# miuda-ai/lele

Hardware: AMD Instinct MI355X
Metric: STFT+mel GB/s (SenseVoice front-end: PCM -> log-mel -> LFR, algorithmic bytes); SenseVoiceSmall-shaped RTF in `sensevoice` (higher is better)
Workload: dtype f32

## Files before the change

### lele_amd/csrc/fe_core.h

```cpp
#pragma once
#include <stdint.h>

#if defined(__HIPCC__)
#define FE_HD __host__ __device__ __forceinline__
#else
#define FE_HD inline
#endif

namespace fe {

constexpr int kNfft = 512;
constexpr int kFrame = 400;
constexpr int kHop = 160;
constexpr int kBins = 257;
constexpr int kLanes = 16;
constexpr int kRegs = 32;
constexpr int kQ = 25;

FE_HD constexpr int rev4(int x) { return ((x & 1) << 3) | ((x & 2) << 1) | ((x & 4) >> 1) | ((x & 8) >> 3); }
FE_HD constexpr int rev5(int x) {
    return ((x & 1) << 4) | ((x & 2) << 2) | (x & 4) | ((x & 8) >> 2) | ((x & 16) >> 4);
}
FE_HD constexpr int tw_off(int s) { return (1 << (s - 1)) - 1; }

FE_HD float fmul(float a, float b) { return a * b; }
FE_HD float fadd(float a, float b) { return a + b; }
FE_HD float fsub(float a, float b) { return a - b; }
FE_HD float ffma(float a, float b, float c) { return __builtin_fmaf(a, b, c); }

#if defined(__HIPCC__) && defined(__HIP_DEVICE_COMPILE__)
typedef float cf __attribute__((ext_vector_type(2)));
FE_HD cf cmk(float re, float im) { return (cf){re, im}; }
FE_HD cf cadd(cf a, cf b) { return a + b; }
FE_HD cf csub(cf a, cf b) { return a - b; }
FE_HD cf cmulv(cf a, cf b) { return a * b; }
FE_HD cf cfmav(cf a, cf b, cf c) { return __builtin_elementwise_fma(a, b, c); }
FE_HD cf cswap(cf a) { return a.yx; }
FE_HD cf cxx(cf a) { return a.xx; }
#else
struct cf {
    float x, y;
};
FE_HD cf cmk(float re, float im) { return cf{re, im}; }
FE_HD cf cadd(cf a, cf b) { return cf{a.x + b.x, a.y + b.y}; }
FE_HD cf csub(cf a, cf b) { return cf{a.x - b.x, a.y - b.y}; }
FE_HD cf cmulv(cf a, cf b) { return cf{a.x * b.x, a.y * b.y}; }
FE_HD cf cfmav(cf a, cf b, cf c) { return cf{__builtin_fmaf(a.x, b.x, c.x), __builtin_fmaf(a.y, b.y, c.y)}; }
FE_HD cf cswap(cf a) { return cf{a.y, a.x}; }
FE_HD cf cxx(cf a) { return cf{a.x, a.x}; }
#endif

struct Tw {
    cf w, wn;
};
FE_HD Tw make_tw(float wr, float wi) { return Tw{cmk(wr, wi), cmk(-wi, wi)}; }

FE_HD cf tw_mul_fma(const Tw& t, cf o) { return cfmav(cxx(t.w), o, cmulv(t.wn, cswap(o))); }

FE_HD void bfly_fma(const Tw& tw, cf& e, cf& o) {
    cf t = tw_mul_fma(tw, o);
    cf n = csub(e, t);
    e = cadd(e, t);
    o = n;
}
FE_HD void bfly_scalar(float wr, float wi, cf& e, cf& o) {
    float tr = fsub(fmul(wr, o.x), fmul(wi, o.y));
    float ti = fadd(fmul(wr, o.y), fmul(wi, o.x));
    cf t = cmk(tr, ti);
    cf n = csub(e, t);
    e = cadd(e, t);
    o = n;
}
FE_HD void bfly_fma(float wr, float wi, float& er, float& ei, float& o_r, float& oi) {
    cf e = cmk(er, ei), o = cmk(o_r, oi);
    bfly_fma(make_tw(wr, wi), e, o);
    er = e.x;
    ei = e.y;
    o_r = o.x;
    oi = o.y;
}
FE_HD void bfly_scalar(float wr, float wi, float& er, float& ei, float& o_r, float& oi) {
    cf e = cmk(er, ei), o = cmk(o_r, oi);
    bfly_scalar(wr, wi, e, o);
    er = e.x;
    ei = e.y;
    o_r = o.x;
    oi = o.y;
}

template <typename TW>
FE_HD void phase_a(cf* a, const TW& tw_re, const TW& tw_im) {
#pragma unroll
    for (int r = 0; r < kRegs; r += 2) bfly_scalar(tw_re[tw_off(1)], tw_im[tw_off(1)], a[r], a[r + 1]);
#pragma unroll
    for (int b = 0; b < kRegs; b += 4) {
#pragma unroll
        for (int k = 0; k < 2; ++k) bfly_scalar(tw_re[tw_off(2) + k], tw_im[tw_off(2) + k], a[b + k], a[b + 2 + k]);
    }
#pragma unroll
    for (int s = 3; s <= 5; ++s) {
        const int half = 1 << (s - 1);
#pragma unroll
        for (int b = 0; b < kRegs; b += 2 * half) {
#pragma unroll
            for (int k = 0; k < half; ++k)
                bfly_fma(make_tw(tw_re[tw_off(s) + k], tw_im[tw_off(s) + k]), a[b + k], a[b + half + k]);
        }
    }
}

template <typename TW>
FE_HD void phase_a_fast(const float* x, cf* a, const TW& tw_re, const TW& tw_im) {
    float s1[kRegs];
#pragma unroll
    for (int r = 0; r < kRegs; r += 2) {
        if (rev5(r + 1) >= kQ) {
            s1[r] = x[r];
            s1[r + 1] = x[r];
        } else {
            s1[r] = fadd(x[r], x[r + 1]);
            s1[r + 1] = fsub(x[r], x[r + 1]);
        }
    }
    {
        const float wr = tw_re[tw_off(2) + 1], wi = tw_im[tw_off(2) + 1];
#pragma unroll
        for (int b = 0; b < kRegs; b += 4) {
            a[b] = cmk(fadd(s1[b], s1[b + 2]), 0.0f);
            a[b + 2] = cmk(fsub(s1[b], s1[b + 2]), 0.0f);
            const float tr = fmul(wr, s1[b + 3]);
            const float ti = fmul(wi, s1[b + 3]);
            a[b + 1] = cmk(fadd(s1[b + 1], tr), ti);
            a[b + 3] = cmk(fsub(s1[b + 1], tr), -ti);
        }
    }
#pragma unroll
    for (int b = 0; b < kRegs; b += 8) {
#pragma unroll
        for (int k = 0; k < 4; ++k) {
            const float wr = tw_re[tw_off(3) + k], wi = tw_im[tw_off(3) + k];
            if ((k & 1) == 0) {
                const float e = a[b + k].x, o = a[b + 4 + k].x;
                const float tr = fmul(wr, o);
                const float ti = fmul(wi, o);
                a[b + k] = cmk(fadd(e, tr), ti);
                a[b + 4 + k] = cmk(fsub(e, tr), -ti);
            } else {
                bfly_fma(make_tw(wr, wi), a[b + k], a[b + 4 + k]);
            }
        }
    }
#pragma unroll
    for (int s = 4; s <= 5; ++s) {
        const int half = 1 << (s - 1);
#pragma unroll
        for (int b = 0; b < kRegs; b += 2 * half) {
#pragma unroll
            for (int k = 0; k < half; ++k)
                bfly_fma(make_tw(tw_re[tw_off(s) + k], tw_im[tw_off(s) + k]), a[b + k], a[b + half + k]);
        }
    }
}

template <typename TWF>
FE_HD void phase_b(cf* b, int c, int rho, const TWF& twf, float* re256) {
#pragma unroll
    for (int s = 6; s <= 8; ++s) {
        const int hv = 1 << (s - 6);
#pragma unroll
        for (int k = 0; k < hv; ++k) {
            const cf w = twf(tw_off(s) + k * 32 + rho * 16 + c);
            const Tw tw = make_tw(w.x, w.y);
#pragma unroll
            for (int base = 0; base < 16; base += 2 * hv) bfly_fma(tw, b[base + k], b[base + hv + k]);
        }
    }
#pragma unroll
    for (int k = 0; k < 8; ++k) {
        const cf w = twf(tw_off(9) + k * 32 + rho * 16 + c);
        const cf t = tw_mul_fma(make_tw(w.x, w.y), b[8 + k]);
        if (k == 0) *re256 = fsub(b[0].x, t.x);
        b[k] = cadd(b[k], t);
    }
}

FE_HD float power(float re, float im) { return fadd(fmul(re, re), fmul(im, im)); }
FE_HD float power(cf z) {
    cf sq = cmulv(z, z);
    return fadd(sq.x, sq.y);
}

constexpr int kXchgPitch = 17;
FE_HD constexpr int xchg_slot(int v, int c) { return v * kXchgPitch + c; }

}
```

### lele_amd/csrc/frontend.hip

```cpp
#include <type_traits>
#include "common.h"
#include "fe_core.h"

#include <math.h>

#include <algorithm>

using namespace lele;

namespace {

constexpr int kMaxMelRounds = 8;

struct FeDev {
    const float* tw_re;
    const float* tw_im;
    const float2* tw;
    const float* window;
    const float* melw;
    const int* mel_start;
    const int* mel_step_off;
    int mel_rounds;
    int mel_steps;
    int n_mels;
    int lfr_m, lfr_n;
};

struct GridBlock {
    __device__ __forceinline__ unsigned x() const { return blockIdx.x; }
    __device__ __forceinline__ unsigned y() const { return blockIdx.y; }
};
struct SegBlock {
    unsigned bx;
    __device__ __forceinline__ unsigned x() const { return bx; }
    __device__ __forceinline__ unsigned y() const { return 0u; }
};

struct FeSeg {
    int64_t start, len;
    int64_t num_frames, t_lfr;
    int64_t row0;
    int64_t block0;
};

constexpr int kSumRows = 66;
constexpr int kSumPitch = 164;

__global__ __launch_bounds__(64) void fe_frame_sum_kernel(const float* __restrict__ pcm, int64_t utt_stride,
                                                          int64_t pcm_len, int64_t num_frames,
                                                          float* __restrict__ mean_out, int aligned16) {
    __shared__ __attribute__((aligned(16))) float tile[kSumRows * kSumPitch];
    const int lane = threadIdx.x;
    const int64_t f0 = (int64_t)blockIdx.x * 64;
    const float* base = pcm + (int64_t)blockIdx.y * utt_stride;
    const int64_t s0 = f0 * fe::kHop;
    constexpr int kVecPerRow = fe::kHop / 4;
    constexpr int kVecs = kSumRows * kVecPerRow;
    constexpr int kIters = (kVecs + 63) / 64;
    constexpr int kBatch = 14;
    static_assert(kIters % kBatch == 0, "batching");
    for (int b0 = 0; b0 < kIters; b0 += kBatch) {
        float4 st[kBatch];
#pragma unroll
        for (int u = 0; u < kBatch; ++u) {
            const int idx = (b0 + u) * 64 + lane;
            int64_t s = s0 + 4 * (int64_t)idx;
            if (s + 3 >= pcm_len) s = aligned16 ? ((pcm_len - 4) & ~int64_t(3)) : (pcm_len - 4);
            if (s < 0) s = 0;
            const float* src = base + s;
            if (aligned16) {
                st[u] = *reinterpret_cast<const float4*>(src);
            } else {
                st[u] = make_float4(src[0], src[1], src[2], src[3]);
            }
        }
#pragma unroll
        for (int u = 0; u < kBatch; ++u) {
            const int idx = (b0 + u) * 64 + lane;
            if (idx < kVecs) {
                float4 xv = st[u];
                xv.x *= 32768.0f;
                xv.y *= 32768.0f;
                xv.z *= 32768.0f;
                xv.w *= 32768.0f;
                const int row = idx / kVecPerRow, c = idx - row * kVecPerRow;
                *reinterpret_cast<float4*>(&tile[row * kSumPitch + 4 * c]) = xv;
            }
        }
    }
    __syncthreads();
    float sum = 0.0f;
#pragma unroll
    for (int seg = 0; seg < 3; ++seg) {
        const float* rowp = &tile[(lane + seg) * kSumPitch];
        const int nvec = seg < 2 ? kVecPerRow : (fe::kFrame - 2 * fe::kHop) / 4;
#pragma unroll 10
        for (int k = 0; k < nvec; ++k) {
            const float4 r = *reinterpret_cast<const float4*>(rowp + 4 * k);
            sum = sum + r.x;
            sum = sum + r.y;
            sum = sum + r.z;
            sum = sum + r.w;
        }
    }
    const int64_t f = f0 + lane;
    if (f < num_frames) mean_out[(int64_t)blockIdx.y * num_frames + f] = sum / (float)fe::kFrame;
}

constexpr int kFrameXchgFloats = 2 * 16 * fe::kXchgPitch;
constexpr int kWaveLdsFloats = 4 * kFrameXchgFloats;
constexpr int kPStride = 272;

struct TwLds {
    const float2* t;
    __device__ __forceinline__ float2 at(int i) const { return t[i]; }
};

template <int MODE>
__device__ __forceinline__ float lane_rot_prev(float v, int p) {
    if (MODE == 1) {
        return __builtin_bit_cast(float,
                                  __builtin_amdgcn_update_dpp(0, __builtin_bit_cast(int, v), 0x121, 0xf, 0xf, true));
    } else {
        return __shfl(v, (p + 15) & 15, 16);
    }
}

constexpr int kStdMelLen[5] = {3, 4, 6, 10, 17};
constexpr int kStdMelOff[6] = {0, 3, 7, 13, 23, 40};

template <int MODE, bool STDMEL, bool FUSED, int PASSES, bool LOWREG, class Blk>
__device__ __forceinline__ void fe_main_body(const float* __restrict__ pcm, int64_t utt_stride,
                                             int64_t num_frames, int64_t t_lfr,
                                             const float* __restrict__ means, const FeDev& tb,
                                             float* __restrict__ out, float* __restrict__ logmel_out,
                                             int aligned16, float* s_melw, Blk bl) {
    constexpr int FR = 16 * PASSES;
    constexpr int kRows = FR + 2;
    constexpr int kXFloats = FUSED ? (kRows * kSumPitch > 4 * kWaveLdsFloats ? kRows * kSumPitch : 4 * kWaveLdsFloats)
                                   : 4 * kWaveLdsFloats;
    __shared__ float2 s_tw[LOWREG ? 480 : 512];
    __shared__ __attribute__((aligned(16))) float s_x[kXFloats];
    __shared__ float s_mean[64];
    __shared__ int s_mstart[16 * (STDMEL ? 5 : kMaxMelRounds)];
    __shared__ int s_moff[kMaxMelRounds + 1];
    constexpr int kTwBase = LOWREG ? 31 : 0;

    for (int i = threadIdx.x; i < 511 - kTwBase; i += 256) s_tw[i] = tb.tw[i + kTwBase];
    if (!STDMEL)
        for (int i = threadIdx.x; i < tb.mel_steps * 16; i += 256) s_melw[i] = tb.melw[i];
    if (threadIdx.x < tb.mel_rounds * 16) s_mstart[threadIdx.x] = tb.mel_start[threadIdx.x];
    if (threadIdx.x <= tb.mel_rounds) s_moff[threadIdx.x] = tb.mel_step_off[threadIdx.x];
    const int lane = threadIdx.x & 63, wave = threadIdx.x >> 6;
    const int g = lane >> 4, p = lane & 15;
    if (FUSED) {
        const float* ubase = pcm + (int64_t)bl.y() * utt_stride;
        const int64_t s0 = (int64_t)bl.x() * FR * fe::kHop;
        constexpr int kVecPerRow = fe::kHop / 4;
        constexpr int kVecs = kRows * kVecPerRow;
        constexpr int kIters = (kVecs + 255) / 256;
        float4 st[kIters];
#pragma unroll
        for (int u = 0; u < kIters; ++u) {
            const int idx = u * 256 + (int)threadIdx.x;
            int64_t sidx = s0 + 4 * (int64_t)idx;
            if (sidx + 3 >= utt_stride) sidx = aligned16 ? ((utt_stride - 4) & ~int64_t(3)) : (utt_stride - 4);
            if (sidx < 0) sidx = 0;
            const float* src = ubase + sidx;
            if (aligned16)
                st[u] = *reinterpret_cast<const float4*>(src);
            else
                st[u] = make_float4(src[0], src[1], src[2], src[3]);
        }
#pragma unroll
        for (int u = 0; u < kIters; ++u) {
            const int idx = u * 256 + (int)threadIdx.x;
            if (idx < kVecs) {
                float4 xv = st[u];
                xv.x *= 32768.0f;
                xv.y *= 32768.0f;
                xv.z *= 32768.0f;
                xv.w *= 32768.0f;
                const int row = idx / kVecPerRow, c = idx - row * kVecPerRow;
                *reinterpret_cast<float4*>(&s_x[row * kSumPitch + 4 * c]) = xv;
            }
        }
        __syncthreads();
    }
    const int h = fe::rev4(p);
    float* xw = s_x + wave * kWaveLdsFloats;
    float* xf = xw + g * kFrameXchgFloats;
    const float* base = pcm + (int64_t)bl.y() * utt_stride;
    const float* mean_u = means + (int64_t)bl.y() * num_frames;
    const int d_out = tb.n_mels * tb.lfr_m;
    float* out_u = out ? out + (int64_t)bl.y() * t_lfr * d_out : nullptr;
    float* lm_u = logmel_out ? logmel_out + (int64_t)bl.y() * num_frames * tb.n_mels : nullptr;

    float win[fe::kQ];
    if (!LOWREG) {
#pragma unroll
        for (int q = 0; q < fe::kQ; ++q) win[q] = tb.window[p + 16 * q];
    }

    float xr[fe::kQ];
    float mean_next = 0.0f;
    auto issue_loads = [&](int pass) {
        const int64_t f = (int64_t)bl.x() * FR + wave * (4 * PASSES) + pass * 4 + g;
        const int64_t fc = f < num_frames ? f : 0;
        const float* src = base + fc * fe::kHop + p;
        if (!FUSED) mean_next = mean_u[fc];
#pragma unroll
        for (int q = 0; q < fe::kQ; ++q) xr[q] = src[16 * q];
    };
    issue_loads(0);
    if (FUSED) {
        constexpr int kVecPerRow = fe::kHop / 4;
        if (wave == 0 && lane < FR) {
            float sum = 0.0f;
#pragma unroll
            for (int seg = 0; seg < 3; ++seg) {
                const float* rowp = &s_x[(lane + seg) * kSumPitch];
                const int nvec = seg < 2 ? kVecPerRow : (fe::kFrame - 2 * fe::kHop) / 4;
#pragma unroll 10
                for (int k = 0; k < nvec; ++k) {
                    const float4 r = *reinterpret_cast<const float4*>(rowp + 4 * k);
                    sum = sum + r.x;
                    sum = sum + r.y;
                    sum = sum + r.z;
                    sum = sum + r.w;
                }
            }
            s_mean[lane] = sum / (float)fe::kFrame;
        }
    }
    __syncthreads();

    auto run_pass = [&](int pass, auto load_next_c) {
        constexpr bool load_next = decltype(load_next_c)::value;
        const int64_t f = (int64_t)bl.x() * FR + wave * (4 * PASSES) + pass * 4 + g;
        const bool valid = f < num_frames;
        const float mean = FUSED ? s_mean[wave * (4 * PASSES) + pass * 4 + g] : mean_next;
        if (LOWREG) {
            int off = 0;
            asm volatile("" : "+v"(off));
#pragma unroll
            for (int q = 0; q < fe::kQ; ++q) win[q] = tb.window[p + 16 * q + off];
        }

        float v[fe::kQ];
        const float neg_mean = -mean;
#pragma unroll
        for (int q = 0; q < fe::kQ; ++q) v[q] = __builtin_fmaf(xr[q], 32768.0f, neg_mean);
        if (load_next) issue_loads(pass + 1);
        float xin[fe::kRegs];
#pragma unroll
        for (int r = 0; r < fe::kRegs; ++r) xin[r] = 0.0f;
        float k97;
        asm("v_mov_b32 %0, 0x3f7851ec" : "=v"(k97));
#pragma unroll
        for (int q = 0; q < fe::kQ; ++q) {
            const float send = (p == 15 && q > 0) ? v[q > 0 ? q - 1 : 0] : v[q];
            const float prev = lane_rot_prev<MODE>(send, p);
            float y = fe::fsub(v[q], fe::fmul(k97, prev));
            if (q == 0) y = (p == 0) ? v[0] : y;
            xin[fe::rev5(q)] = fe::fmul(y, win[q]);
        }

        fe::cf a[fe::kRegs];
        fe::phase_a_fast(xin, a, tb.tw_re, tb.tw_im);

        float pw[2][8];
        float p256 = 0.0f;
#pragma unroll
        for (int rho = 0; rho < 2; ++rho) {
            __builtin_amdgcn_wave_barrier();
#pragma unroll
            for (int cc = 0; cc < 16; ++cc) {
                const int slot = fe::xchg_slot(h, cc);
                *reinterpret_cast<float2*>(xf + 2 * slot) = make_float2(a[rho * 16 + cc].x, a[rho * 16 + cc].y);
            }
            __builtin_amdgcn_wave_barrier();
            fe::cf bq[16];
#pragma unroll
            for (int vv = 0; vv < 16; ++vv) {
                const float2 t = *reinterpret_cast<const float2*>(xf + 2 * fe::xchg_slot(vv, p));
                bq[vv] = fe::cmk(t.x, t.y);
            }
            __builtin_amdgcn_wave_barrier();
            float re256 = 0.0f;
            fe::phase_b(bq, p, rho, [&](int i) { const float2 w = s_tw[i - kTwBase]; return fe::cmk(w.x, w.y); }, &re256);
            if (rho == 0) p256 = re256;
#pragma unroll
            for (int vv = 0; vv < 8; ++vv) {
                fe::cf z = bq[vv];
                if (vv == 0 && rho == 0) z = fe::cmk(z.x, (p == 0) ? 0.0f : z.y);
                pw[rho][vv] = fe::power(z);
            }
        }
        float* prow = xw + g * kPStride;
        __builtin_amdgcn_wave_barrier();
#pragma unroll
        for (int rho = 0; rho < 2; ++rho)
#pragma unroll
            for (int vv = 0; vv < 8; ++vv) prow[(2 * vv + rho) * 16 + p] = pw[rho][vv];
        if (p == 0) prow[256] = fe::power(p256, 0.0f);
        __builtin_amdgcn_wave_barrier();

        const int fi = (int)f, nfr = (int)num_frames, tl = (int)t_lfr;
        const int pad = (tb.lfr_m - 1) / 2;
        const int fp = fi + pad;
        const int b_first = fp % tb.lfr_n, i_first = fp / tb.lfr_n;

        float vals[STDMEL ? 5 : kMaxMelRounds];
#pragma unroll
        for (int rd = 0; rd < (STDMEL ? 5 : kMaxMelRounds); ++rd) {
            vals[rd] = 0.0f;
            if (!STDMEL && rd >= tb.mel_rounds) continue;
            const int m = rd * 16 + p;
            const int start = s_mstart[m];
            const float* pp = prow + start;
            float acc = 0.0f;
            if (STDMEL) {
                const float* wp = tb.melw + kStdMelOff[rd < 5 ? rd : 0] * 16 + p;
                float w[17];
#pragma unroll
                for (int t = 0; t < 17; ++t)
                    if (t < kStdMelLen[rd < 5 ? rd : 0]) w[t] = wp[t * 16];
#pragma unroll
                for (int t = 0; t < 17; ++t)
                    if (t < kStdMelLen[rd < 5 ? rd : 0]) acc = fe::fadd(acc, fe::fmul(w[t], pp[t]));
            } else {
                const int t0 = s_moff[rd], t1 = s_moff[rd + 1];
                const float* wp = s_melw + t0 * 16 + p;
                const int lim = 256 - start;
#pragma unroll 4
                for (int t = 0; t < t1 - t0; ++t) {
                    const float pv = pp[t < lim ? t : lim];
                    acc = fe::fadd(acc, fe::fmul(wp[t * 16], pv));
                }
            }
            {
                const float l2 = __builtin_amdgcn_logf(fmaxf(acc, 1e-5f));
                const float hi = __builtin_bit_cast(float, 0x3f317217u), lo = __builtin_bit_cast(float, 0x3377d1cfu);
                const float r = fe::fmul(l2, hi);
                vals[rd] = fe::fadd(r, fe::ffma(l2, lo, fe::ffma(l2, hi, -r)));
            }
        }
        if (valid) {
            constexpr int kR = STDMEL ? 5 : kMaxMelRounds;
            auto put = [&](float* dst) {
#pragma unroll
                for (int rd = 0; rd < kR; ++rd)
                    if (rd * 16 + p < tb.n_mels) __builtin_nontemporal_store(vals[rd], &dst[rd * 16]);
            };
            if (lm_u) put(lm_u + (int64_t)fi * tb.n_mels + p);
            if (out_u) {
                int i = i_first;
                for (int b = b_first; b < tb.lfr_m && i >= 0; b += tb.lfr_n, --i)
                    if (i < tl) put(out_u + i * d_out + b * tb.n_mels + p);
                if (fi == 0) {
                    for (int i2 = 0; i2 * tb.lfr_n - pad < 0 && i2 < tl; ++i2)
                        for (int b = 0; b < tb.lfr_m && i2 * tb.lfr_n + b - pad < 0; ++b)
                            put(out_u + i2 * d_out + b * tb.n_mels + p);
                }
                if (fi == nfr - 1) {
                    for (int i2 = tl - 1; i2 >= 0 && i2 * tb.lfr_n + (tb.lfr_m - 1) - pad > fi; --i2)
                        for (int b = tb.lfr_m - 1; b >= 0 && i2 * tb.lfr_n + b - pad > fi; --b)
                            put(out_u + i2 * d_out + b * tb.n_mels + p);
                }
            }
        }
        __builtin_amdgcn_wave_barrier();
    };
#pragma unroll 1
    for (int pass = 0; pass + 1 < PASSES; ++pass) run_pass(pass, std::true_type{});
    run_pass(PASSES - 1, std::false_type{});
}

template <int MODE, bool STDMEL, bool FUSED>
__global__ __launch_bounds__(256) void fe_main_kernel(const float* __restrict__ pcm, int64_t utt_stride, int64_t num_frames, int64_t t_lfr,
                                                      const float* __restrict__ means, FeDev tb, float* __restrict__ out,
                                                      float* __restrict__ logmel_out, int aligned16) {
    extern __shared__ float s_melw[];
    fe_main_body<MODE, STDMEL, FUSED, 4, false>(pcm, utt_stride, num_frames, t_lfr, means, tb, out, logmel_out, aligned16, s_melw,
                                                GridBlock{});
}

template <int MODE, bool STDMEL>
__global__ __launch_bounds__(256) void fe_seg_main_kernel(const float* __restrict__ pcm, const FeSeg* __restrict__ segs,
                                                          const int* __restrict__ blk_seg, FeDev tb, float* __restrict__ out) {
    extern __shared__ float s_melw[];
    const FeSeg s = segs[blk_seg[blockIdx.x]];
    const float* base = pcm + s.start;
    const int aligned16 = (((uintptr_t)base & 15) == 0) && (s.len % 4 == 0);
    fe_main_body<MODE, STDMEL, true, 4, false>(base, s.len, s.num_frames, s.t_lfr, nullptr, tb, out + s.row0 * (tb.n_mels * tb.lfr_m),
                                               nullptr, aligned16, s_melw, SegBlock{(unsigned)(blockIdx.x - s.block0)});
}
__global__ void fe_generic_mean_kernel(const float* __restrict__ pcm, int64_t rows, int64_t num_frames, int64_t pcm_len, int frame_len, int hop,
                                       float* __restrict__ mean) {
    const int64_t f = (int64_t)blockIdx.x * blockDim.x + threadIdx.x;
    if (f >= rows) return;
    const float* src = pcm + (f / num_frames) * pcm_len + (f % num_frames) * hop;
    float sum = 0.0f;
    int j = 0;
    if ((((uintptr_t)src) & 15) == 0) {
        for (; j + 16 <= frame_len; j += 16) {
            float4 v[4];
#pragma unroll
            for (int u = 0; u < 4; ++u) v[u] = *reinterpret_cast<const float4*>(src + j + 4 * u);
#pragma unroll
            for (int u = 0; u < 4; ++u) {
                sum = sum + v[u].x * 32768.0f;
                sum = sum + v[u].y * 32768.0f;
                sum = sum + v[u].z * 32768.0f;
                sum = sum + v[u].w * 32768.0f;
            }
        }
    }
    for (; j < frame_len; ++j) sum = sum + src[j] * 32768.0f;
    mean[f] = sum / (float)frame_len;
}
__global__ void fe_generic_frame_kernel(const float* __restrict__ pcm, const float* __restrict__ mean,
                                        const float* __restrict__ window, int64_t rows, int64_t num_frames, int64_t pcm_len, int frame_len, int hop,
                                        int n_fft, float* __restrict__ frames) {
    const int64_t total = rows * n_fft;
    for (int64_t i = (int64_t)blockIdx.x * blockDim.x + threadIdx.x; i < total; i += (int64_t)gridDim.x * blockDim.x) {
        const int64_t f = i / n_fft;
        const int j = (int)(i - f * n_fft);
        float v = 0.0f;
        if (j < frame_len) {
            const float* src = pcm + (f / num_frames) * pcm_len + (f % num_frames) * hop;
            const float m = mean[f];
            const float cur = fe::fsub(fe::fmul(src[j], 32768.0f), m);
            float y = cur;
            if (j >= 1) y = fe::fsub(cur, fe::fmul(0.97f, fe::fsub(fe::fmul(src[j - 1], 32768.0f), m)));
            v = fe::fmul(y, window[j]);
        }
        frames[i] = v;
    }
}
__global__ void fe_generic_mel_kernel(const float* __restrict__ power, int64_t num_frames, int n_bins, int n_mels,
                                      const int* __restrict__ mstart, const int* __restrict__ moff,
                                      const float* __restrict__ mw, float* __restrict__ logmel) {
    const int64_t total = num_frames * n_mels;
    for (int64_t i = (int64_t)blockIdx.x * blockDim.x + threadIdx.x; i < total; i += (int64_t)gridDim.x * blockDim.x) {
        const int64_t f = i / n_mels;
        const int m = (int)(i - f * n_mels);
        const float* p = power + f * n_bins + mstart[m];
        float acc = 0.0f;
        for (int t = moff[m]; t < moff[m + 1]; ++t) acc = fe::fadd(acc, fe::fmul(mw[t], p[t - moff[m]]));
        logmel[i] = __logf(fmaxf(acc, 1e-5f));
    }
}
#define FE_PAD(i) ((i) + ((i) >> 5))
__global__ __launch_bounds__(256) void fe_generic_fused_kernel(const float* __restrict__ pcm, int64_t pcm_len, int64_t num_frames, int frame_len,
                                                               int hop, int n, int log2n, int fpb, const float* __restrict__ window,
                                                               const float* __restrict__ tw_re_g, const float* __restrict__ tw_im_g, int n_mels,
                                                               const int* __restrict__ mstart, const int* __restrict__ moff,
                                                               const float* __restrict__ mw, const float* __restrict__ means,
                                                               float* __restrict__ logmel) {
    extern __shared__ float gfl[];
    const int nb = n / 2 + 1, span = (fpb - 1) * hop + frame_len;
    float* re = gfl;
    float* im = re + FE_PAD(fpb * n) + 1;
    float* pw = im + FE_PAD(fpb * n) + 1;
    float* sp = pw + fpb * nb;
    float* smean = sp + span;
    const int tid = threadIdx.x;
    const int64_t f0 = (int64_t)blockIdx.x * fpb;
    const int nfr = (int)(num_frames - f0 < fpb ? num_frames - f0 : fpb);
    const float* src = pcm + (int64_t)blockIdx.y * pcm_len + f0 * hop;
    const int have = (nfr - 1) * hop + frame_len;
    for (int i = tid; i < span; i += 256) sp[i] = i < have ? src[i] : 0.0f;
    __syncthreads();
    if (means) {
        if (tid < nfr) smean[tid] = means[(int64_t)blockIdx.y * num_frames + f0 + tid];
    } else if (tid < nfr) {
        const float* fr = sp + tid * hop;
        float sum = 0.0f;
        int j = 0;
        for (; j + 16 <= frame_len; j += 16) {
            float v[16];
#pragma unroll
            for (int u = 0; u < 16; ++u) v[u] = fr[j + u];
#pragma unroll
            for (int u = 0; u < 16; ++u) sum = sum + v[u] * 32768.0f;
        }
        for (; j < frame_len; ++j) sum = sum + fr[j] * 32768.0f;
        smean[tid] = sum / (float)frame_len;
    }
    __syncthreads();
    for (int i = tid; i < fpb * n; i += 256) {
        const int f = i >> log2n, j = i & (n - 1);
        float v = 0.0f;
        if (j < frame_len && f < nfr) {
            const float* fr = sp + f * hop;
            const float m = smean[f];
            const float cur = fe::fsub(fe::fmul(fr[j], 32768.0f), m);
            float y = cur;
            if (j >= 1) y = fe::fsub(cur, fe::fmul(0.97f, fe::fsub(fe::fmul(fr[j - 1], 32768.0f), m)));
            v = fe::fmul(y, window[j]);
        }
        const int r = (int)(__brev((unsigned)j) >> (32 - log2n));
        re[FE_PAD(f * n + r)] = v;
        im[FE_PAD(f * n + r)] = 0.0f;
    }
    __syncthreads();
    for (int s0 = 0; s0 < log2n;) {
        const int R = log2n - s0 >= 3 ? 3 : log2n - s0, h = 1 << s0, gsz = 1 << R, groups = n >> R;
        for (int idx = tid; idx < fpb * groups; idx += 256) {
            const int f = idx / groups, g = idx - f * groups;
            const int lo = g & (h - 1), base = f * n + ((g >> s0) << (s0 + R)) + lo;
            float xr[8], xi[8];
#pragma unroll
            for (int j = 0; j < 8; ++j)
                if (j < gsz) xr[j] = re[FE_PAD(base + j * h)], xi[j] = im[FE_PAD(base + j * h)];
#pragma unroll
            for (int r = 0; r < 3; ++r) {
                if (r >= R) break;
                const int half = h << r, off = half - 1;
#pragma unroll
                for (int j = 0; j < 8; ++j) {
                    if (j >= gsz || (j >> r) & 1) continue;
                    const int k = lo + (j & ((1 << r) - 1)) * h;
                    const float wr = tw_re_g[off + k], wi = tw_im_g[off + k];
                    if (half >= 4)
                        fe::bfly_fma(wr, wi, xr[j], xi[j], xr[j + (1 << r)], xi[j + (1 << r)]);
                    else
                        fe::bfly_scalar(wr, wi, xr[j], xi[j], xr[j + (1 << r)], xi[j + (1 << r)]);
                }
            }
#pragma unroll
            for (int j = 0; j < 8; ++j)
                if (j < gsz) re[FE_PAD(base + j * h)] = xr[j], im[FE_PAD(base + j * h)] = xi[j];
        }
        s0 += R;
        __syncthreads();
    }
    for (int i = tid; i < fpb * nb; i += 256) {
        const int f = i / nb, k = i - f * nb;
        const float r = re[FE_PAD(f * n + k)];
        const float q = (k == 0 || k == nb - 1) ? 0.0f : im[FE_PAD(f * n + k)];
        pw[i] = fe::power(r, q);
    }
    __syncthreads();
    for (int i = tid; i < nfr * n_mels; i += 256) {
        const int f = i / n_mels, m = i - f * n_mels;
        const float* pp = pw + f * nb + mstart[m];
        const float* wp = mw + moff[m];
        const int cnt = moff[m + 1] - moff[m];
        float acc = 0.0f;
        int t = 0;
        for (; t + 8 <= cnt; t += 8) {
            float w8[8], p8[8];
#pragma unroll
            for (int u = 0; u < 8; ++u) w8[u] = wp[t + u], p8[u] = pp[t + u];
#pragma unroll
            for (int u = 0; u < 8; ++u) acc = fe::fadd(acc, fe::fmul(w8[u], p8[u]));
        }
        for (; t < cnt; ++t) acc = fe::fadd(acc, fe::fmul(wp[t], pp[t]));
        logmel[((int64_t)blockIdx.y * num_frames + f0 + f) * n_mels + m] = __logf(fmaxf(acc, 1e-5f));
    }
}
__global__ void fe_generic_lfr_kernel(const float* __restrict__ x, int64_t t, int64_t d, int64_t m, int64_t n,
                                      int64_t t_lfr, float* __restrict__ out) {
    const int64_t d_out = d * m, total = t_lfr * d_out, pad = (m - 1) / 2;
    x += (int64_t)blockIdx.y * t * d;
    out += (int64_t)blockIdx.y * total;
    for (int64_t idx = (int64_t)blockIdx.x * blockDim.x + threadIdx.x; idx < total; idx += (int64_t)gridDim.x * blockDim.x) {
        const int64_t i = idx / d_out, rem = idx - i * d_out, block = rem / d, k = rem - block * d;
        int64_t raw = i * n + block - pad;
        raw = raw < 0 ? 0 : (raw > t - 1 ? t - 1 : raw);
        out[idx] = x[raw * d + k];
    }
}

}

struct LeleFrontend {
    LeleCtx* ctx = nullptr;
    LeleFeatureConfig cfg{};
    int64_t frame_len = 0, hop_len = 0, n_fft = 0;
    bool fast = false;
    bool std_mel = false;
    int dpp_mode = 0;
    bool fused = true;
    const float* g_window = nullptr;
    const int* g_mstart = nullptr;
    const int* g_moff = nullptr;
    const float* g_mw = nullptr;
    FeDev dev{};
    std::vector<void*> allocs;
    DevTables seg_tables;
    bool profiling = false;
    std::vector<hipEvent_t> events;
    size_t events_used = 0;
};

namespace {

static const float PI_F = 3.14159265358979323846264338327950288f;

void host_hann(int64_t size, std::vector<float>& w) {
    w.resize(size);
    if (size == 1) w[0] = 1.0f;
    for (int64_t n = 0; size > 1 && n < size; ++n) w[n] = 0.5f * (1.0f - cosf(2.0f * PI_F * (float)n / (float)(size - 1)));
}

void host_twiddles(int64_t n, std::vector<float>& re, std::vector<float>& im) {
    re.clear();
    im.clear();
    for (int64_t size = 2; size <= n; size *= 2) {
        int64_t half = size / 2, step = n / size;
        for (int64_t k = 0; k < half; ++k) {
            float angle = -2.0f * PI_F * (float)(k * step) / (float)n;
            re.push_back(cosf(angle));
            im.push_back(sinf(angle));
        }
    }
}

float hz_to_mel(float hz) { return 2595.0f * log10f(1.0f + hz / 700.0f); }
float mel_to_hz(float mel) { return 700.0f * (powf(10.0f, mel / 2595.0f) - 1.0f); }

void host_dense_mel(float sr, int64_t n_fft, int64_t n_mels, float f_min, float f_max, float* bank) {
    const int64_t n_freqs = n_fft / 2 + 1;
    const float mel_min = hz_to_mel(f_min), mel_max = hz_to_mel(f_max);
    const float mel_step = (mel_max - mel_min) / (float)(n_mels + 1);
    std::vector<float> hz(n_mels + 2), ff(n_freqs);
    for (int64_t i = 0; i < n_mels + 2; ++i) hz[i] = mel_to_hz(mel_min + (float)i * mel_step);
    for (int64_t i = 0; i < n_freqs; ++i) ff[i] = (float)i * sr / (float)n_fft;
    for (int64_t i = 0; i < n_mels; ++i) {
        const float fl = hz[i], fc = hz[i + 1], fr = hz[i + 2];
        for (int64_t j = 0; j < n_freqs; ++j) {
            const float f = ff[j];
            float val = 0.0f;
            if (f > fl && f < fc)
                val = (f - fl) / (fc - fl);
            else if (f >= fc && f < fr)
                val = (fr - f) / (fr - fc);
            bank[i * n_freqs + j] = val;
        }
    }
}

void host_sparse_mel(float sr, int64_t n_fft, int64_t n_mels, float f_min, std::vector<int>& start,
                     std::vector<std::vector<float>>& w) {
    const int64_t n_freqs = n_fft / 2 + 1;
    std::vector<float> bank((size_t)n_mels * n_freqs);
    host_dense_mel(sr, n_fft, n_mels, f_min, sr / 2.0f, bank.data());
// ... 481 lines not shown
```

Before: 1833.

## Batch twiddle LDS loads and restructure phase-B exchange schedule in STFT kernel

Refactors phase_b into per-twiddle steps so twiddle loads from shared memory can be issued in batches ahead of the butterflies, with sched_barrier fences forcing the load/compute grouping. The two rho halves are unrolled explicitly, reusing the upper half of the register array as the second buffer. Mel-filter start indices are hoisted into registers once per block, and the fused mean value is prefetched for the next pass. The aim is to hide LDS latency and cut redundant shared-memory reads, at the cost of more live registers.

```diff
diff --git a/lele_amd/csrc/fe_core.h b/lele_amd/csrc/fe_core.h
--- a/lele_amd/csrc/fe_core.h
+++ b/lele_amd/csrc/fe_core.h
@@ -162,26 +162,30 @@
     }
 }
 
+constexpr int kTwB = 15;
+constexpr int kTwB0 = 31;
+FE_HD constexpr int tw_b_index(int i, int rho, int c) { return kTwB0 + 32 * i + rho * 16 + c; }
+
+FE_HD void phase_b_tw(cf* b, int i, cf w, float* re256) {
+    const Tw tw = make_tw(w.x, w.y);
+    if (i < 7) {
+        const int s = i < 1 ? 6 : i < 3 ? 7 : 8;
+        const int hv = 1 << (s - 6);
+        const int k = i - (hv - 1);
+#pragma unroll
+        for (int base = 0; base < 16; base += 2 * hv) bfly_fma(tw, b[base + k], b[base + hv + k]);
+    } else {
+        const int k = i - 7;
+        const cf t = tw_mul_fma(tw, b[8 + k]);
+        if (k == 0) *re256 = fsub(b[0].x, t.x);
+        b[k] = cadd(b[k], t);
+    }
+}
+
 template <typename TWF>
 FE_HD void phase_b(cf* b, int c, int rho, const TWF& twf, float* re256) {
 #pragma unroll
-    for (int s = 6; s <= 8; ++s) {
-        const int hv = 1 << (s - 6);
-#pragma unroll
-        for (int k = 0; k < hv; ++k) {
-            const cf w = twf(tw_off(s) + k * 32 + rho * 16 + c);
-            const Tw tw = make_tw(w.x, w.y);
-#pragma unroll
-            for (int base = 0; base < 16; base += 2 * hv) bfly_fma(tw, b[base + k], b[base + hv + k]);
-        }
-    }
-#pragma unroll
-    for (int k = 0; k < 8; ++k) {
-        const cf w = twf(tw_off(9) + k * 32 + rho * 16 + c);
-        const cf t = tw_mul_fma(make_tw(w.x, w.y), b[8 + k]);
-        if (k == 0) *re256 = fsub(b[0].x, t.x);
-        b[k] = cadd(b[k], t);
-    }
+    for (int i = 0; i < kTwB; ++i) phase_b_tw(b, i, twf(tw_b_index(i, rho, c)), re256);
 }
 
 FE_HD float power(float re, float im) { return fadd(fmul(re, re), fmul(im, im)); }
diff --git a/lele_amd/csrc/frontend.hip b/lele_amd/csrc/frontend.hip
--- a/lele_amd/csrc/frontend.hip
+++ b/lele_amd/csrc/frontend.hip
@@ -234,12 +234,18 @@
         }
     }
     __syncthreads();
+    int mstart[5] = {0, 0, 0, 0, 0};
+    if (STDMEL) {
+#pragma unroll
+        for (int rd = 0; rd < 5; ++rd) mstart[rd] = s_mstart[rd * 16 + p];
+    }
+    if (FUSED) mean_next = s_mean[wave * (4 * PASSES) + g];
 
     auto run_pass = [&](int pass, auto load_next_c) {
         constexpr bool load_next = decltype(load_next_c)::value;
         const int64_t f = (int64_t)bl.x() * FR + wave * (4 * PASSES) + pass * 4 + g;
         const bool valid = f < num_frames;
-        const float mean = FUSED ? s_mean[wave * (4 * PASSES) + pass * 4 + g] : mean_next;
+        const float mean = mean_next;
         if (LOWREG) {
             int off = 0;
             asm volatile("" : "+v"(off));
@@ -269,34 +275,62 @@
         fe::cf a[fe::kRegs];
         fe::phase_a_fast(xin, a, tb.tw_re, tb.tw_im);
 
-        float pw[2][8];
-        float p256 = 0.0f;
-#pragma unroll
-        for (int rho = 0; rho < 2; ++rho) {
-            __builtin_amdgcn_wave_barrier();
-#pragma unroll
-            for (int cc = 0; cc < 16; ++cc) {
-                const int slot = fe::xchg_slot(h, cc);
-                *reinterpret_cast<float2*>(xf + 2 * slot) = make_float2(a[rho * 16 + cc].x, a[rho * 16 + cc].y);
-            }
-            __builtin_amdgcn_wave_barrier();
-            fe::cf bq[16];
+        auto xchg_write = [&](const fe::cf* src) {
+#pragma unroll
+            for (int cc = 0; cc < 16; ++cc)
+                *reinterpret_cast<float2*>(xf + 2 * fe::xchg_slot(h, cc)) = make_float2(src[cc].x, src[cc].y);
+        };
+        auto xchg_read = [&](fe::cf* dst) {
 #pragma unroll
             for (int vv = 0; vv < 16; ++vv) {
                 const float2 t = *reinterpret_cast<const float2*>(xf + 2 * fe::xchg_slot(vv, p));
-                bq[vv] = fe::cmk(t.x, t.y);
-            }
-            __builtin_amdgcn_wave_barrier();
-            float re256 = 0.0f;
-            fe::phase_b(bq, p, rho, [&](int i) { const float2 w = s_tw[i - kTwBase]; return fe::cmk(w.x, w.y); }, &re256);
-            if (rho == 0) p256 = re256;
+                dst[vv] = fe::cmk(t.x, t.y);
+            }
+        };
+        auto tw_read = [&](fe::cf* tw, int rho, int i0, int i1) {
+#pragma unroll
+            for (int i = i0; i < i1; ++i) {
+                const float2 w = s_tw[fe::tw_b_index(i, rho, p) - kTwBase];
+                tw[i] = fe::cmk(w.x, w.y);
+            }
+        };
+        float pw[2][8];
+        auto powers = [&](const fe::cf* bq, int rho) {
 #pragma unroll
             for (int vv = 0; vv < 8; ++vv) {
                 fe::cf z = bq[vv];
                 if (vv == 0 && rho == 0) z = fe::cmk(z.x, (p == 0) ? 0.0f : z.y);
                 pw[rho][vv] = fe::power(z);
             }
-        }
+        };
+        constexpr int kTwBatch = 3;
+        float p256 = 0.0f, re256 = 0.0f;
+        fe::cf bq0[16], tw0[fe::kTwB], tw1[fe::kTwB];
+        fe::cf* bq1 = a + 16;
+        __builtin_amdgcn_wave_barrier();
+        xchg_write(a);
+        __builtin_amdgcn_wave_barrier();
+        xchg_read(bq0);
+#pragma unroll
+        for (int i0 = 0; i0 < fe::kTwB; i0 += kTwBatch) {
+            constexpr int kB = kTwBatch;
+            const int i1 = i0 + kB < fe::kTwB ? i0 + kB : fe::kTwB;
+            tw_read(tw0, 0, i0, i1);
+            __builtin_amdgcn_sched_barrier(0);
+#pragma unroll
+            for (int i = i0; i < i1; ++i) fe::phase_b_tw(bq0, i, tw0[i], &p256);
+        }
+        powers(bq0, 0);
+        __builtin_amdgcn_wave_barrier();
+        xchg_write(a + 16);
+        __builtin_amdgcn_wave_barrier();
+        xchg_read(bq1);
+        tw_read(tw1, 1, 0, fe::kTwB);
+        __builtin_amdgcn_wave_barrier();
+        __builtin_amdgcn_sched_barrier(0);
+#pragma unroll
+        for (int i = 0; i < fe::kTwB; ++i) fe::phase_b_tw(bq1, i, tw1[i], &re256);
+        powers(bq1, 1);
         float* prow = xw + g * kPStride;
         __builtin_amdgcn_wave_barrier();
 #pragma unroll
@@ -316,8 +350,7 @@
         for (int rd = 0; rd < (STDMEL ? 5 : kMaxMelRounds); ++rd) {
             vals[rd] = 0.0f;
             if (!STDMEL && rd >= tb.mel_rounds) continue;
-            const int m = rd * 16 + p;
-            const int start = s_mstart[m];
+            const int start = STDMEL ? mstart[rd < 5 ? rd : 0] : s_mstart[rd * 16 + p];
             const float* pp = prow + start;
             float acc = 0.0f;
             if (STDMEL) {
@@ -346,6 +379,7 @@
                 vals[rd] = fe::fadd(r, fe::ffma(l2, lo, fe::ffma(l2, hi, -r)));
             }
         }
+        if (FUSED && load_next) mean_next = s_mean[wave * (4 * PASSES) + (pass + 1) * 4 + g];
         if (valid) {
             constexpr int kR = STDMEL ? 5 : kMaxMelRounds;
             auto put = [&](float* dst) {
```

After: 1839, median of 6. No clear change (+0.4%).
